# jaak-s/libfastsparse

Measured on AMD Instinct MI355X. Metric: fp64 CSR SpMV effective GB/s (% HBM3E peak), higher is better.
Workload: dtype f64

## Files before the change

libfastsparse_amd/csrc/fs_kernels_twopass.hip:

```cpp
#include <stdlib.h>

#include "fs_kernel_util.h"

namespace fs {


template <int U, bool NTLD, bool NTST, int BC>
__device__ __forceinline__ void expand_share(double *__restrict__ xband, int ncol, int B, const unsigned *__restrict__ band_ptr,
                                             const uint16_t *__restrict__ lcol, const unsigned *__restrict__ gdst,
                                             const double *__restrict__ x, int xs, double *__restrict__ prod, unsigned g0,
                                             unsigned g1)
{
  const int t = threadIdx.x;
  if (g0 >= g1) return;
  int b;
  {
    int lo = 0, hi = B - 1;
    while (lo < hi) {
      const int mid = lo + ((hi - lo + 1) >> 1);
      if (band_ptr[mid] <= g0) lo = mid; else hi = mid - 1;
    }
    b = lo;
  }
  for (unsigned g = g0; g < g1; ++b) {
    const unsigned gb = band_ptr[b + 1] < g1 ? band_ptr[b + 1] : g1;
    if (gb <= g) continue;
    const int c0 = b * BC;
    const int w = (ncol - c0 < BC) ? ncol - c0 : BC;
    __syncthreads();
    {
      double r[BC / kBinBlock];
#pragma unroll
      for (int j = 0; j < BC / kBinBlock; ++j) {
        const int i = j * kBinBlock + t;
        r[j] = __builtin_nontemporal_load(x + (int64_t)(c0 + (i < w ? i : w - 1)) * xs);
      }
#pragma unroll
      for (int j = 0; j < BC / kBinBlock; ++j) {
        const int i = j * kBinBlock + t;
        xband[i] = (i < w) ? r[j] : 0.0;
      }
      if (t < 8) xband[BC + t] = 0.0;
    }
    __syncthreads();
    const int64_t e0 = (int64_t)g * kBinGroup, e1 = (int64_t)gb * kBinGroup;
    constexpr int64_t kRound = 2 * U * kBinBlock;
    int64_t o = e0 + 2 * t;
    for (; o - 2 * t + kRound <= e1; o += kRound) {
      unsigned a[U], d[U];
#pragma unroll
      for (int k = 0; k < U; ++k) {
        const int64_t e = o + (int64_t)k * 2 * kBinBlock;
        a[k] = stream_load<NTLD>((const unsigned *)(lcol + e));
        d[k] = stream_load<NTLD>(gdst + (e >> kBinGroupLog));
      }
      __builtin_amdgcn_sched_barrier(0);
#pragma unroll
      for (int k = 0; k < U; ++k) {
        const int64_t e = o + (int64_t)k * 2 * kBinBlock;
        const v2d p = {xband[a[k] & 0xffffu], xband[a[k] >> 16]};
        stream_store<NTST>(p, (v2d *)(prod + (int64_t)d[k] * kBinGroup + (e & (kBinGroup - 1))));
      }
    }
    for (; o < e1; o += 2 * kBinBlock) {
      const unsigned a = stream_load<NTLD>((const unsigned *)(lcol + o));
      const unsigned d = stream_load<NTLD>(gdst + (o >> kBinGroupLog));
      const v2d p = {xband[a & 0xffffu], xband[a >> 16]};
      stream_store<NTST>(p, (v2d *)(prod + (int64_t)d * kBinGroup + (o & (kBinGroup - 1))));
    }
    g = gb;
  }
}

template <int U, bool NTLD, bool NTST, int BC = kBinCols>
__global__ __launch_bounds__(kBinBlock) void spmv_expand_kernel(
    int ncol, int B, const unsigned *__restrict__ band_ptr, const uint16_t *__restrict__ lcol,
    const unsigned *__restrict__ gdst, const double *__restrict__ x, int xs, double *__restrict__ prod, unsigned gbeg,
    unsigned gend)
{
  __shared__ double xband[BC + 8];
  const uint64_t groups = gend - gbeg;
  const unsigned g0 = gbeg + (unsigned)(groups * blockIdx.x / gridDim.x), g1 = gbeg + (unsigned)(groups * (blockIdx.x + 1) / gridDim.x);
  expand_share<U, NTLD, NTST, BC>(xband, ncol, B, band_ptr, lcol, gdst, x, xs, prod, g0, g1);
}

static_assert(kBinGroupLog == 4, "the one-byte row ids (row_ids, line_ids, rows8_decode_kernel) decode groups of 16 entries: two lanes of 8, eight lanes of 2, four words of 4");
template <bool NTLD, bool L8>
__device__ __forceinline__ v4u row_ids_load(const uint16_t *__restrict__ lrow, const uint8_t *__restrict__ lrow8,
                                            const uint16_t *__restrict__ gbase, int64_t e)
{
  if (!L8) return stream_load<NTLD>((const v4u *)(lrow + e));
  typedef unsigned v2u __attribute__((ext_vector_type(2)));
  const v2u d = stream_load<NTLD>((const v2u *)(lrow8 + e));
  return v4u{d.x, d.y, (unsigned)gbase[e >> kBinGroupLog], (unsigned)(e >> 3) & 1u};
}

template <bool L8>
__device__ __forceinline__ v4u row_ids(v4u raw)
{
  if (!L8) return raw;
  const unsigned dx = raw.x, dy = raw.y;
  const unsigned s0 = dx & 0xffu, s1 = s0 + ((dx >> 8) & 0xffu), s2 = s1 + ((dx >> 16) & 0xffu), s3 = s2 + (dx >> 24);
  const unsigned s4 = s3 + (dy & 0xffu), s5 = s4 + ((dy >> 8) & 0xffu), s6 = s5 + ((dy >> 16) & 0xffu), s7 = s6 + (dy >> 24);
  const unsigned below = (unsigned)__builtin_amdgcn_update_dpp(0, (int)s7, 0x111 , 0xf, 0xf, false);
  const unsigned off = raw.z + (raw.w ? below : 0u);
  return v4u{(off + s0) | ((off + s1) << 16), (off + s2) | ((off + s3) << 16), (off + s4) | ((off + s5) << 16), (off + s6) | ((off + s7) << 16)};
}

template <bool L8>
__device__ __forceinline__ unsigned line_ids_load(const uint16_t *__restrict__ lrow, const uint8_t *__restrict__ lrow8,
                                                  const uint16_t *__restrict__ gbase, int64_t e)
{
  if (!L8) return *(const unsigned *)(lrow + e);
  return (unsigned)*(const uint16_t *)(lrow8 + e) | ((unsigned)gbase[e >> kBinGroupLog] << 16);
}

template <bool L8>
__device__ __forceinline__ unsigned line_ids(unsigned raw)
{
  if (!L8) return raw;
  const unsigned d0 = raw & 0xffu, own = d0 + ((raw >> 8) & 0xffu), l = threadIdx.x & 7u;
  unsigned s = own, u;
  u = (unsigned)__builtin_amdgcn_update_dpp(0, (int)s, 0x111 , 0xf, 0xf, false); s += l >= 1 ? u : 0u;
  u = (unsigned)__builtin_amdgcn_update_dpp(0, (int)s, 0x112 , 0xf, 0xf, false); s += l >= 2 ? u : 0u;
  u = (unsigned)__builtin_amdgcn_update_dpp(0, (int)s, 0x114 , 0xf, 0xf, false); s += l >= 4 ? u : 0u;
  const unsigned off = (raw >> 16) + s - own;
  return (off + d0) | ((off + own) << 16);
}

template <bool VALUED, bool NTLD, bool L8 = false>
__device__ __forceinline__ void reduce_panel(double *__restrict__ ytile, int panel, const unsigned *__restrict__ bin_ptr,
                                             const int *__restrict__ panel_row, const uint16_t *__restrict__ lrow,
                                             const double *__restrict__ vals, const double *__restrict__ prod, double *__restrict__ y,
                                             int ys, const uint8_t *__restrict__ lrow8 = nullptr,
                                             const uint16_t *__restrict__ gbase = nullptr)
{
  const int t = threadIdx.x;
  const int r0 = panel_row[panel], nr = panel_row[panel + 1] - r0;
  for (int i = t; i < nr; i += kBinBlock) ytile[i] = 0.0;
  __syncthreads();
  const int64_t e0 = (int64_t)bin_ptr[panel] * kBinGroup, e1 = (int64_t)bin_ptr[panel + 1] * kBinGroup;
#define FS_ADD(idx, val) __hip_atomic_fetch_add(&ytile[idx], val, __ATOMIC_RELAXED, __HIP_MEMORY_SCOPE_WORKGROUP)
#define FS_ADD2(A, P) FS_ADD((A) & 0xffffu, (P).x); FS_ADD((A) >> 16, (P).y);
  constexpr int64_t kStep = 8 * kBinBlock, kRound = 2 * kStep;
  const int wave0 = (t >> 6) * 512, lane0 = wave0 + 2 * (t & 63);
  int64_t eb = e0;
  for (; eb + kRound <= e1; eb += kRound) {
    const int64_t e = eb + lane0;
    unsigned a[2][4];
    v2d p[2][4], v[2][4];
#pragma unroll
    for (int k = 0; k < 2; ++k)
#pragma unroll
      for (int j = 0; j < 4; ++j) {
        const int64_t ek = e + k * kStep + 128 * j;
        a[k][j] = line_ids_load<L8>(lrow, lrow8, gbase, ek);
        p[k][j] = stream_load<NTLD>((const v2d *)(prod + ek));
        if (VALUED) v[k][j] = stream_load<NTLD>((const v2d *)(vals + ek));
      }
    __builtin_amdgcn_sched_barrier(0);
#pragma unroll
    for (int k = 0; k < 2; ++k)
#pragma unroll
      for (int j = 0; j < 4; ++j) {
        const unsigned r = line_ids<L8>(a[k][j]);
        if (VALUED) { p[k][j].x *= v[k][j].x; p[k][j].y *= v[k][j].y; }
        FS_ADD2(r, p[k][j])
      }
  }
  for (; eb + wave0 < e1; eb += kStep) {
    const int64_t e = eb + lane0;
    unsigned a[4];
    v2d p[4], v[4];
#pragma unroll
    for (int j = 0; j < 4; ++j) {
      const int64_t ej = e + 128 * j, ec = ej < e1 ? ej : e1 - 2;
      a[j] = line_ids_load<L8>(lrow, lrow8, gbase, ec);
      p[j] = stream_load<NTLD>((const v2d *)(prod + ec));
      if (VALUED) v[j] = stream_load<NTLD>((const v2d *)(vals + ec));
    }
#pragma unroll
    for (int j = 0; j < 4; ++j) {
      const unsigned r = line_ids<L8>(a[j]);
      if (VALUED) { p[j].x *= v[j].x; p[j].y *= v[j].y; }
      if (e + 128 * j < e1) { FS_ADD2(r, p[j]) }
    }
  }
#undef FS_ADD2
#undef FS_ADD
  __syncthreads();
  for (int i = t; i < nr; i += kBinBlock) y[(int64_t)(r0 + i) * ys] = ytile[i];
}

template <bool VALUED, bool NTLD, int RM = kBinRowsMax, bool L8 = false>
__global__ __launch_bounds__(kBinBlock) void spmv_reduce_kernel(
    const unsigned *__restrict__ bin_ptr, const int *__restrict__ panel_row, const uint16_t *__restrict__ lrow,
    const double *__restrict__ vals, const double *__restrict__ prod, double *__restrict__ y, int ys, int pbase,
    const uint8_t *__restrict__ lrow8 = nullptr, const uint16_t *__restrict__ gbase = nullptr)
{
  __shared__ double ytile[RM];
  reduce_panel<VALUED, NTLD, L8>(ytile, pbase + blockIdx.x, bin_ptr, panel_row, lrow, vals, prod, y, ys, lrow8, gbase);
}

#ifndef FS_ORDERED_DEPTH
#define FS_ORDERED_DEPTH 16
#endif
#ifndef FS_ORDERED_DEPTH_VALUED
#define FS_ORDERED_DEPTH_VALUED 10
#endif
template <bool VALUED, bool NTLD, int RM, int DEPTH, bool L8 = false>
__global__ __launch_bounds__(64) void spmv_reduce_ordered_kernel(
    const unsigned *__restrict__ bin_ptr, const int *__restrict__ panel_row, const uint16_t *__restrict__ lrow,
    const double *__restrict__ vals, const double *__restrict__ prod, double *__restrict__ y, int ys, int pbase,
    const uint8_t *__restrict__ lrow8 = nullptr, const uint16_t *__restrict__ gbase = nullptr)
{
  __shared__ __attribute__((aligned(16))) double ytile[RM];
  const int t = threadIdx.x;
  const int panel = pbase + blockIdx.x;
  const int r0 = panel_row[panel], nr = panel_row[panel + 1] - r0;
  for (int i = 2 * t; i < nr; i += 128) *reinterpret_cast<v2d *>(&ytile[i]) = v2d{0.0, 0.0};
  const int64_t e0 = (int64_t)bin_ptr[panel] * kBinGroup, e1 = (int64_t)bin_ptr[panel + 1] * kBinGroup;
#define FS_ADD(idx, val) __hip_atomic_fetch_add(&ytile[idx], val, __ATOMIC_RELAXED, __HIP_MEMORY_SCOPE_WORKGROUP)
#define FS_ADD8(A, P)                                                  \
  FS_ADD(A.x & 0xffffu, P[0].x); FS_ADD(A.x >> 16, P[0].y);            \
  FS_ADD(A.y & 0xffffu, P[1].x); FS_ADD(A.y >> 16, P[1].y);            \
  FS_ADD(A.z & 0xffffu, P[2].x); FS_ADD(A.z >> 16, P[2].y);            \
  FS_ADD(A.w & 0xffffu, P[3].x); FS_ADD(A.w >> 16, P[3].y);
  constexpr int64_t kStep = 8 * 64;
  v4u a[DEPTH];
  v2d p[DEPTH][4], v[VALUED ? DEPTH : 1][4];
  auto fetch = [&](int k, int64_t e) {
    const int64_t ec = (e + 8 <= e1) ? e : (e1 - e0 >= 8 ? e1 - 8 : e0);
    a[k] = row_ids_load<NTLD, L8>(lrow, lrow8, gbase, ec);
#pragma unroll
    for (int j = 0; j < 4; ++j) {
      p[k][j] = stream_load<NTLD>((const v2d *)(prod + ec + 2 * j));
      if (VALUED) v[k][j] = stream_load<NTLD>((const v2d *)(vals + ec + 2 * j));
    }
  };
  if (e1 > e0) {
    int64_t e = e0 + 8 * t;
#pragma unroll
    for (int k = 0; k < DEPTH; ++k) fetch(k, e + (int64_t)k * kStep);
    for (; e - 8 * t < e1; e += (int64_t)DEPTH * kStep) {
#pragma unroll
      for (int k = 0; k < DEPTH; ++k) {
        const int64_t ek = e + (int64_t)k * kStep;
        const v4u ak = row_ids<L8>(a[k]);
        v2d pk[4] = {p[k][0], p[k][1], p[k][2], p[k][3]};
        if (VALUED) {
#pragma unroll
          for (int j = 0; j < 4; ++j) { pk[j].x *= v[k][j].x; pk[j].y *= v[k][j].y; }
        }
        fetch(k, ek + (int64_t)DEPTH * kStep);
        if (ek + 8 <= e1) { FS_ADD8(ak, pk) }
      }
    }
  }
#undef FS_ADD8
#undef FS_ADD
  __syncthreads();
  for (int i = t; i < nr; i += 64) y[(int64_t)(r0 + i) * ys] = ytile[i];
}

template <bool VALUED, int BC, int NACC, bool ORDERED>
__global__ __launch_bounds__(kBinBlock) void spmv_longrows_kernel(
    int ncol, int B, int nlong, const int64_t *__restrict__ band_ptr, const unsigned *__restrict__ seg_ptr,
    const uint16_t *__restrict__ lcol, const uint16_t *__restrict__ lrow, const double *__restrict__ vals,
    const double *__restrict__ x, int xs, double *__restrict__ ylong, double *__restrict__ ypart)
{
  __shared__ double xband[BC + 8];
  __shared__ double acc[NACC];
  const int t = threadIdx.x, lane = t & 63, wave = t >> 6;
  for (int i = t; i < nlong; i += kBinBlock) acc[i] = 0.0;
  const int64_t pairs = band_ptr[B] >> 1;
  const int64_t e_beg = 2 * (pairs * blockIdx.x / gridDim.x), e_end = 2 * (pairs * (blockIdx.x + 1) / gridDim.x);
  if (e_beg < e_end) {
    int b;
    {
      int lo = 0, hi = B - 1;
      while (lo < hi) {
        const int mid = lo + ((hi - lo + 1) >> 1);
        if (band_ptr[mid] <= e_beg) lo = mid; else hi = mid - 1;
      }
      b = lo;
    }
    double rn[BC / kBinBlock];
    int have = -1;
    auto request = [&](int bb) {
      const int cb = bb * BC;
      const int wb = (ncol - cb < BC) ? ncol - cb : BC;
#pragma unroll
      for (int j = 0; j < BC / kBinBlock; ++j) {
        const int i = j * kBinBlock + t;
        rn[j] = __builtin_nontemporal_load(x + (int64_t)(cb + (i < wb ? i : wb - 1)) * xs);
      }
      have = bb;
    };
    auto wave_step = [&](int64_t o, bool live, int64_t oc) {
      const unsigned a = *reinterpret_cast<const unsigned *>(lcol + oc);
      const unsigned rr = *reinterpret_cast<const unsigned *>(lrow + oc);
      v2d p = {xband[a & 0xffffu], xband[a >> 16]};
      if (VALUED) { const v2d v = *reinterpret_cast<const v2d *>(vals + oc); p.x *= v.x; p.y *= v.y; }
      unsigned key = 0xffffffffu;
      double sum = 0.0;
      if (live) {
        const unsigned r0 = rr & 0xffffu, r1 = rr >> 16;
        if (r0 == r1) { key = r0; sum = p.x + p.y; }
        else { __hip_atomic_fetch_add(&acc[r0], p.x, __ATOMIC_RELAXED, __HIP_MEMORY_SCOPE_WORKGROUP); key = r1; sum = p.y; }
      }
#pragma unroll
      for (int d = 1; d < 64; d <<= 1) {
        const unsigned ku = __shfl_up(key, d);
        const double su = __shfl_up(sum, d);
        if (lane >= d && ku == key) sum += su;
      }
      const unsigned kn = __shfl_down(key, 1);
      if (live && (lane == 63 || kn != key))
        __hip_atomic_fetch_add(&acc[key], sum, __ATOMIC_RELAXED, __HIP_MEMORY_SCOPE_WORKGROUP);
      (void)o;
    };
    for (int64_t e = e_beg; e < e_end; ++b) {
      const int64_t eb = band_ptr[b + 1] < e_end ? band_ptr[b + 1] : e_end;
      if (eb <= e) continue;
      const int c0 = b * BC;
      const int w = (ncol - c0 < BC) ? ncol - c0 : BC;
      if (have != b) request(b);
      __syncthreads();
#pragma unroll
      for (int j = 0; j < BC / kBinBlock; ++j) {
        const int i = j * kBinBlock + t;
        xband[i] = (i < w) ? rn[j] : 0.0;
      }
      if (t < 8) xband[BC + t] = 0.0;
      __syncthreads();
      if (b + 1 < B && eb < e_end) request(b + 1);
      if (ORDERED) {
        const int64_t s0 = band_ptr[b] + seg_ptr[b * (kLongOwners + 1) + wave], s1 = band_ptr[b] + seg_ptr[b * (kLongOwners + 1) + wave + 1];
        const int64_t lo = s0 > e ? s0 : e, hi = s1 < eb ? s1 : eb;
        for (int64_t o0 = lo; o0 < hi; o0 += 128) {
          const int64_t o = o0 + 2 * lane;
          const bool live = o < hi;
          wave_step(o, live, live ? o : lo);
        }
      } else {
        for (int64_t o0 = e; o0 < eb; o0 += 2 * kBinBlock) {
          const int64_t o = o0 + 2 * t;
          const bool live = o < eb;
          wave_step(o, live, live ? o : e);
        }
      }
      e = eb;
    }
  }
  __syncthreads();
  if (ORDERED) {
    double *__restrict__ mine = ypart + (int64_t)blockIdx.x * nlong;
    for (int i = t; i < nlong; i += kBinBlock) mine[i] = acc[i];
  } else {
    for (int i = t; i < nlong; i += kBinBlock) {
      const double v = acc[i];
      if (v != 0.0) unsafeAtomicAdd(ylong + i, v);
    }
  }
}

__global__ __launch_bounds__(kBlock) void longrows_combine_kernel(int nlong, int nwg, const double *__restrict__ ypart, double *__restrict__ ylong)
{
  const int i = blockIdx.x * kBlock + threadIdx.x;
  if (i >= nlong) return;
  double acc = 0.0;
  for (int w = 0; w < nwg; ++w) acc += ypart[(int64_t)w * nlong + i];
  ylong[i] = acc;
}

__global__ __launch_bounds__(kBlock) void longrows_scatter_kernel(int nlong, const int *__restrict__ row, const double *__restrict__ ylong,
                                                                 double *__restrict__ y, int ys, int row0, int row1)
{
  const int i = blockIdx.x * kBlock + threadIdx.x;
  if (i >= nlong) return;
  const int r = row[i];
  if (r >= row0 && r < row1) y[(int64_t)r * ys] = 0.0 + ylong[i];
}

static int launch_longrows(const DeviceCsr &A, const LongRows &L, const double *x, int xs, hipStream_t s)
{
  const bool ordered = reproducible_now();
  if (!ordered || L.n == 0 || L.nwg == 0)
    if (int rc = launch_zero(L.ylong, sizeof(double) * (size_t)L.nlong, s)) return rc;
  if (L.n == 0 || L.nwg == 0) return FS_OK;
#define FS_LONG(V, BC, NA, ORD)                                                                                              \
  hipLaunchKernelGGL((spmv_longrows_kernel<V, BC, NA, ORD>), dim3(L.nwg), dim3(kBinBlock), 0, s, A.ncol, L.B, L.nlong, L.band_ptr, \
                     L.seg_ptr, L.lcol, L.lrow, L.vals, x, xs, L.ylong, L.ypart)
#define FS_LONG2(V, BC, NA) do { if (ordered) FS_LONG(V, BC, NA, true); else FS_LONG(V, BC, NA, false); } while (0)
  if (L.bcols == kLongBandB) { if (A.has_vals()) FS_LONG2(true, kLongBandB, kLongRowsB); else FS_LONG2(false, kLongBandB, kLongRowsB); }
  else                       { if (A.has_vals()) FS_LONG2(true, kLongBandA, kLongRowsA); else FS_LONG2(false, kLongBandA, kLongRowsA); }
#undef FS_LONG2
#undef FS_LONG
  FS_HIP(hipGetLastError());
  if (ordered) {
    hipLaunchKernelGGL(longrows_combine_kernel, dim3((unsigned)((L.nlong + kBlock - 1) / kBlock)), dim3(kBlock), 0, s, L.nlong, L.nwg, L.ypart,
                       L.ylong);
    FS_HIP(hipGetLastError());
  }
  return FS_OK;
}


template <int K, int U>
__global__ __launch_bounds__(kBinBlock) void spmm_expand_kernel(
    int ncol, int B, const unsigned *__restrict__ band_ptr, const uint16_t *__restrict__ lcol,
    const unsigned *__restrict__ gdst, const double *__restrict__ X, int xs, double *__restrict__ prod)
{
  constexpr int BC = kBinCols / K;
  constexpr int GE = kBinGroup / K;
  constexpr int LP = K / 2;
  constexpr int EPS = kBinBlock / LP;
  __shared__ __attribute__((aligned(16))) double xband[kBinCols + 8];
  const int t = threadIdx.x;
  const int le = t / LP, h = t % LP;
  const uint64_t groups = band_ptr[B];
  const unsigned g0 = (unsigned)(groups * blockIdx.x / gridDim.x), g1 = (unsigned)(groups * (blockIdx.x + 1) / gridDim.x);
  if (g0 >= g1) return;
  int b;
  {
    int lo = 0, hi = B - 1;
    while (lo < hi) {
      const int mid = lo + ((hi - lo + 1) >> 1);
      if (band_ptr[mid] <= g0) lo = mid; else hi = mid - 1;
    }
    b = lo;
  }
  for (unsigned g = g0; g < g1; ++b) {
    const unsigned gb = band_ptr[b + 1] < g1 ? band_ptr[b + 1] : g1;
    if (gb <= g) continue;
    const int c0 = b * BC;
    const int w = (ncol - c0 < BC) ? ncol - c0 : BC;
    __syncthreads();
    {
      double r[kBinCols / kBinBlock];
#pragma unroll
      for (int j = 0; j < kBinCols / kBinBlock; ++j) {
        const int f = j * kBinBlock + t, i = f / K, q = f % K;
        r[j] = __builtin_nontemporal_load(X + (int64_t)(c0 + (i < w ? i : w - 1)) * xs + q);
      }
#pragma unroll
      for (int j = 0; j < kBinCols / kBinBlock; ++j) {
        const int f = j * kBinBlock + t;
        xband[f] = (f / K < w) ? r[j] : 0.0;
      }
      if (t < 8) xband[kBinCols + t] = 0.0;
    }
    __syncthreads();
    const int64_t e0 = (int64_t)g * GE, e1 = (int64_t)gb * GE;
    constexpr int64_t kRound = (int64_t)U * EPS;
    int64_t o = e0 + le;
    for (; o - le + kRound <= e1; o += kRound) {
      unsigned a[U], d[U];
#pragma unroll
      for (int k = 0; k < U; ++k) {
        const int64_t e = o + (int64_t)k * EPS;
        a[k] = lcol[e];
        d[k] = gdst[e / GE];
      }
      __builtin_amdgcn_sched_barrier(0);
#pragma unroll
      for (int k = 0; k < U; ++k) {
        const int64_t e = o + (int64_t)k * EPS;
        const v2d p = *reinterpret_cast<const v2d *>(&xband[a[k] * K + 2 * h]);
        __builtin_nontemporal_store(p, (v2d *)(prod + ((int64_t)d[k] * GE + (e % GE)) * K + 2 * h));
      }
    }
    for (; o < e1; o += EPS) {
      const unsigned a = lcol[o];
      const unsigned d = gdst[o / GE];
      const v2d p = *reinterpret_cast<const v2d *>(&xband[a * K + 2 * h]);
      __builtin_nontemporal_store(p, (v2d *)(prod + ((int64_t)d * GE + (o % GE)) * K + 2 * h));
    }
    g = gb;
  }
}

template <bool VALUED, int K>
__global__ __launch_bounds__(kBinBlock) void spmm_reduce_kernel(
    const unsigned *__restrict__ bin_ptr_all, const int *__restrict__ panel_row_all, const uint16_t *__restrict__ lrow,
    const double *__restrict__ vals, const double *__restrict__ prod, double *__restrict__ Y, int ys, int pbase)
{
  const unsigned *__restrict__ bin_ptr = bin_ptr_all + pbase;
  const int *__restrict__ panel_row = panel_row_all + pbase;
  constexpr int GE = kBinGroup / K;
  constexpr int EPL = 8 / K;
  __shared__ double ytile[kBinRowsMax];
  const int t = threadIdx.x;
  const int r0 = panel_row[blockIdx.x], nr = panel_row[blockIdx.x + 1] - r0;
  for (int i = t; i < nr * K; i += kBinBlock) ytile[i] = 0.0;
  __syncthreads();
  const int64_t e0 = (int64_t)bin_ptr[blockIdx.x] * GE, e1 = (int64_t)bin_ptr[blockIdx.x + 1] * GE;
  typedef uint16_t rows_t __attribute__((ext_vector_type(EPL)));
  typedef double vals_t __attribute__((ext_vector_type(EPL)));
#define FS_ADD(idx, val) __hip_atomic_fetch_add(&ytile[idx], val, __ATOMIC_RELAXED, __HIP_MEMORY_SCOPE_WORKGROUP)
  auto add8 = [&](const rows_t a, const v2d (&p)[4], const vals_t v) {
#pragma unroll
    for (int q = 0; q < EPL; ++q) {
      const int base = (int)a[q] * K;
#pragma unroll
      for (int j = 0; j < K; j += 2) {
        v2d t2 = p[(q * K + j) / 2];
        if (VALUED) { t2.x *= v[q]; t2.y *= v[q]; }
        FS_ADD(base + j, t2.x);
        FS_ADD(base + j + 1, t2.y);
      }
    }
  };
  constexpr int64_t kStep = (int64_t)EPL * kBinBlock;
  constexpr int64_t kRound = 2 * kStep;
  int64_t e = e0 + (int64_t)EPL * t;
  for (; e - EPL * t + kRound <= e1; e += kRound) {
    rows_t a[2];
    v2d p[2][4];
    vals_t v[2] = {};
#pragma unroll
    for (int k = 0; k < 2; ++k) {
      const int64_t ek = e + k * kStep;
      a[k] = *reinterpret_cast<const rows_t *>(lrow + ek);
      if (VALUED) v[k] = *reinterpret_cast<const vals_t *>(vals + ek);
#pragma unroll
      for (int j = 0; j < 4; ++j) p[k][j] = *reinterpret_cast<const v2d *>(prod + ek * K + 2 * j);
    }
    __builtin_amdgcn_sched_barrier(0);
    add8(a[0], p[0], v[0]);
    add8(a[1], p[1], v[1]);
  }
  for (; e < e1; e += kStep) {
    const rows_t a = *reinterpret_cast<const rows_t *>(lrow + e);
    vals_t v = {};
    if (VALUED) v = *reinterpret_cast<const vals_t *>(vals + e);
    v2d p[4];
#pragma unroll
    for (int j = 0; j < 4; ++j) p[j] = *reinterpret_cast<const v2d *>(prod + e * K + 2 * j);
    add8(a, p, v);
  }
#undef FS_ADD
  __syncthreads();
  for (int i = t; i < nr * K; i += kBinBlock) Y[(int64_t)(r0 + i / K) * ys + (i % K)] = ytile[i];
}

template <bool VALUED, int K, int DEPTH>
__global__ __launch_bounds__(64) void spmm_reduce_ordered_kernel(
    const unsigned *__restrict__ bin_ptr_all, const int *__restrict__ panel_row_all, const uint16_t *__restrict__ lrow,
    const double *__restrict__ vals, const double *__restrict__ prod, double *__restrict__ Y, int ys, int pbase)
{
  const unsigned *__restrict__ bin_ptr = bin_ptr_all + pbase;
  const int *__restrict__ panel_row = panel_row_all + pbase;
  constexpr int GE = kBinGroup / K;
  constexpr int EPL = 8 / K;
  __shared__ double ytile[kBinRowsMax];
  const int t = threadIdx.x;
  const int r0 = panel_row[blockIdx.x], nr = panel_row[blockIdx.x + 1] - r0;
  for (int i = t; i < nr * K; i += 64) ytile[i] = 0.0;
  const int64_t e0 = (int64_t)bin_ptr[blockIdx.x] * GE, e1 = (int64_t)bin_ptr[blockIdx.x + 1] * GE;
  typedef uint16_t rows_t __attribute__((ext_vector_type(EPL)));
  typedef double vals_t __attribute__((ext_vector_type(EPL)));
#define FS_ADD(idx, val) __hip_atomic_fetch_add(&ytile[idx], val, __ATOMIC_RELAXED, __HIP_MEMORY_SCOPE_WORKGROUP)
  auto add8 = [&](const rows_t a, const v2d (&p)[4], const vals_t v) {
#pragma unroll
    for (int q = 0; q < EPL; ++q) {
      const int base = (int)a[q] * K;
#pragma unroll
      for (int j = 0; j < K; j += 2) {
        v2d t2 = p[(q * K + j) / 2];
        if (VALUED) { t2.x *= v[q]; t2.y *= v[q]; }
        FS_ADD(base + j, t2.x);
        FS_ADD(base + j + 1, t2.y);
      }
    }
  };
  constexpr int64_t kStep = (int64_t)EPL * 64;
  rows_t a[DEPTH];
  v2d p[DEPTH][4];
  vals_t v[VALUED ? DEPTH : 1] = {};
  auto fetch = [&](int k, int64_t e) {
    const int64_t ec = (e + EPL <= e1) ? e : (e1 - e0 >= EPL ? e1 - EPL : e0);
    a[k] = *reinterpret_cast<const rows_t *>(lrow + ec);
    if (VALUED) v[k] = *reinterpret_cast<const vals_t *>(vals + ec);
#pragma unroll
    for (int j = 0; j < 4; ++j) p[k][j] = *reinterpret_cast<const v2d *>(prod + ec * K + 2 * j);
  };
  if (e1 > e0) {
    int64_t e = e0 + (int64_t)EPL * t;
#pragma unroll
    for (int k = 0; k < DEPTH; ++k) fetch(k, e + (int64_t)k * kStep);
    for (; e - EPL * t < e1; e += (int64_t)DEPTH * kStep) {
#pragma unroll
      for (int k = 0; k < DEPTH; ++k) {
        const int64_t ek = e + (int64_t)k * kStep;
        const rows_t ak = a[k];
        const v2d pk[4] = {p[k][0], p[k][1], p[k][2], p[k][3]};
        const vals_t vk = v[VALUED ? k : 0];
        fetch(k, ek + (int64_t)DEPTH * kStep);
        if (ek + EPL <= e1) add8(ak, pk, vk);
      }
    }
  }
#undef FS_ADD
  __syncthreads();
  for (int i = t; i < nr * K; i += 64) Y[(int64_t)(r0 + i / K) * ys + (i % K)] = ytile[i];
}

template <int K>
__global__ __launch_bounds__(kBlock) void tiled_combine_k_kernel(int nrow, const int *__restrict__ vfirst,
                                                                const double *__restrict__ yv, double *__restrict__ Y, int ys,
                                                                int row0 = 0)
{
  const int64_t i = (int64_t)row0 * K + (int64_t)blockIdx.x * kBlock + threadIdx.x;
  const int64_t r = i / K;
  const int j = (int)(i % K);
  if (r >= nrow) return;
  const int a = vfirst[r], b = vfirst[r + 1];
  double acc = yv[(int64_t)a * K + j];
  for (int v = a + 1; v < b; ++v) acc += yv[(int64_t)v * K + j];
  Y[r * ys + j] = acc;
}

__global__ void rows8_decode_kernel(int64_t groups, const uint8_t *__restrict__ lrow8, const uint16_t *__restrict__ gbase,
                                    uint16_t *__restrict__ lrow)
{
  const int64_t g = (int64_t)blockIdx.x * blockDim.x + threadIdx.x;
  if (g >= groups) return;
  const v4u d = *(const v4u *)(lrow8 + g * kBinGroup);
  unsigned r = gbase[g];
  unsigned out[kBinGroup / 2];
#pragma unroll
  for (int j = 0; j < kBinGroup; j += 2) {
    const unsigned w = j < 4 ? d.x : j < 8 ? d.y : j < 12 ? d.z : d.w;
    const unsigned a = r + ((w >> (8 * (j & 3))) & 0xffu), b = a + ((w >> (8 * ((j + 1) & 3))) & 0xffu);
    out[j / 2] = a | (b << 16);
    r = b;
  }
#pragma unroll
  for (int j = 0; j < kBinGroup / 8; ++j)
    *(v4u *)(lrow + g * kBinGroup + 8 * j) = v4u{out[4 * j], out[4 * j + 1], out[4 * j + 2], out[4 * j + 3]};
}

static void ensure_two_byte_ids(BinnedCsr &N, hipStream_t s)
{
  if (N.lrow || !N.lrow8 || N.lrow_tried) return;
  hipStreamCaptureStatus cap = hipStreamCaptureStatusNone;
  if (hipStreamIsCapturing(s, &cap) != hipSuccess) { (void)hipGetLastError(); return; }
  if (cap != hipStreamCaptureStatusNone) return;
  N.lrow_tried = true;
  uint16_t *p = nullptr;
  if (hipMalloc(&p, sizeof(uint16_t) * (size_t)N.n) != hipSuccess) { (void)hipGetLastError(); return; }
  const int64_t groups = N.n >> kBinGroupLog;
  if (groups > 0) hipLaunchKernelGGL(rows8_decode_kernel, dim3((unsigned)((groups + 255) / 256)), dim3(256), 0, s, groups, N.lrow8, N.gbase, p);
  if (hipGetLastError() != hipSuccess || hipStreamSynchronize(s) != hipSuccess) { (void)hipGetLastError(); (void)hipFree(p); return; }
  N.lrow = p;
}

static void launch_reduce(const BinnedCsr &N, double *out, int os, int p0, int p1, int flags, hipStream_t s)
{
#define FS_REDUCE(V, NT, RM, L8)                                                                                                \
  hipLaunchKernelGGL((spmv_reduce_kernel<V, NT, RM, L8>), dim3(p1 - p0), dim3(kBinBlock), 0, s, N.bin_ptr, N.panel_row, N.lrow, \
                     N.vals, N.prod, out, os, p0, N.lrow8, N.gbase)
#define FS_REDUCE2(RM, L8)                                                                       \
  do {                                                                                           \
    if (N.vals) { if (flags & 256) FS_REDUCE(true, false, RM, L8); else FS_REDUCE(true, true, RM, L8); }   \
    else        { if (flags & 256) FS_REDUCE(false, false, RM, L8); else FS_REDUCE(false, true, RM, L8); } \
  } while (0)
  if (N.bcols == kBinColsBig) FS_REDUCE2(kBinRowsBig, false);
  else if (N.lrow8)           FS_REDUCE2(kBinRowsMax, true);
  else                        FS_REDUCE2(kBinRowsMax, false);
#undef FS_REDUCE2
#undef FS_REDUCE
}

int launch_spmv_binned(const DeviceCsr &A, double *y, const double *x, hipStream_t s, int xs, int ys, int p0, int p1, int row0,
                       int row1)
{
  const BinnedCsr &N = *A.binned;
  double *out = N.split ? N.yv : y;
  const int os = N.split ? 1 : ys;
  const bool part = p1 >= 0;
  if (!part) { p0 = 0; p1 = N.P; row0 = 0; row1 = A.nrow; }
  const int nwg1 = (options().bin_wgs > 0 && options().bin_wgs < N.nwg1) ? options().bin_wgs : N.nwg1;
  if (nwg1 > 0 && p0 == 0) {
    const int flags = options().bin_flags;
#define FS_EXPAND4(U)                                                                                       \
  do {                                                                                                      \
    if (flags & 16) { if (flags & 8) FS_EXPAND(U, true, false);  else FS_EXPAND(U, true, true); }           \
    else            { if (flags & 8) FS_EXPAND(U, false, false); else FS_EXPAND(U, false, true); }          \
  } while (0)
#define FS_EXPAND(U, NL, NS)                                                                                      \
  hipLaunchKernelGGL((spmv_expand_kernel<U, NL, NS>), dim3(nwg1), dim3(kBinBlock), 0, s, A.ncol, N.B, N.band_ptr, \
                     N.lcol, N.gdst, x, xs, N.prod, 0u, (unsigned)(N.n >> kBinGroupLog))
    if (N.bcols == kBinColsBig)
      hipLaunchKernelGGL((spmv_expand_kernel<4, false, true, kBinColsBig>), dim3(nwg1), dim3(kBinBlock), 0, s, A.ncol, N.B,
                         N.band_ptr, N.lcol, N.gdst, x, xs, N.prod, 0u, (unsigned)(N.n >> kBinGroupLog));
    else if ((flags & 3) == 1) FS_EXPAND4(8);
    else if ((flags & 3) == 2) FS_EXPAND4(2);
    else                       FS_EXPAND4(4);
#undef FS_EXPAND4
#undef FS_EXPAND
    FS_HIP(hipGetLastError());
  }
  if (N.lr && p0 == 0)
    if (int rc = launch_longrows(A, *N.lr, x, xs, s)) return rc;
  if (p1 > p0) {
    const bool ordered = reproducible_now() || (options().bin_flags & 32);
    if (ordered && N.lrow8 && !N.lrow) ensure_two_byte_ids(*A.binned, s);
#define FS_ORDERED(RM, L8)                                                                                                     \
  do {                                                                                                                         \
    if (N.vals)                                                                                                                \
      hipLaunchKernelGGL((spmv_reduce_ordered_kernel<true, false, RM, FS_ORDERED_DEPTH_VALUED, L8>), dim3(p1 - p0), dim3(64), 0, s, \
                         N.bin_ptr, N.panel_row, N.lrow, N.vals, N.prod, out, os, p0, N.lrow8, N.gbase);                       \
    else                                                                                                                       \
      hipLaunchKernelGGL((spmv_reduce_ordered_kernel<false, false, RM, FS_ORDERED_DEPTH, L8>), dim3(p1 - p0), dim3(64), 0, s,  \
                         N.bin_ptr, N.panel_row, N.lrow, N.vals, N.prod, out, os, p0, N.lrow8, N.gbase);                       \
  } while (0)
    if (N.bcols == kBinColsBig && ordered)  FS_ORDERED(kBinRowsBig, false);
    else if (ordered && N.lrow8 && !N.lrow) FS_ORDERED(kBinRowsMax, true);
    else if (ordered)                       FS_ORDERED(kBinRowsMax, false);
    else
      launch_reduce(N, out, os, p0, p1, options().bin_flags, s);
#undef FS_ORDERED
    FS_HIP(hipGetLastError());
  }
  if (N.split && row1 > row0) {
    if (int rc = launch_tiled_combine(row1, N.vfirst, N.yv, y, ys, row0, s)) return rc;
  }
  if (N.lr && row1 > row0) {
    hipLaunchKernelGGL(longrows_scatter_kernel, dim3((unsigned)((N.lr->nlong + kBlock - 1) / kBlock)), dim3(kBlock), 0, s, N.lr->nlong,
                       N.lr->row, N.lr->ylong, y, ys, row0, row1);
    FS_HIP(hipGetLastError());
  }
  return FS_OK;
}

int launch_expand_groups(const DeviceCsr &A, const double *x, unsigned g0, unsigned g1, int wgs, hipStream_t s)
{
  const BinnedCsr &N = *A.binned;
  if (g1 <= g0 || wgs <= 0) return FS_OK;
#define FS_XH(BC)                                                                                                         \
  hipLaunchKernelGGL((spmv_expand_kernel<4, false, true, BC>), dim3(wgs), dim3(kBinBlock), 0, s, A.ncol, N.B, N.band_ptr, \
                     N.lcol, N.gdst, x, 1, N.prod, g0, g1)
  if (N.bcols == kBinColsBig) FS_XH(kBinColsBig);
  else                        FS_XH(kBinCols);
#undef FS_XH
  FS_HIP(hipGetLastError());
  return FS_OK;
}

int launch_reduce_panels(const DeviceCsr &A, double *y, int p0, int p1, hipStream_t s)
{
  const BinnedCsr &N = *A.binned;
  if (p1 <= p0) return FS_OK;
  launch_reduce(N, y, 1, p0, p1, 0, s);
  FS_HIP(hipGetLastError());
  return FS_OK;
}

int launch_spmm_binned(const DeviceCsr &A, const BinnedCsr &N, double *Y, const double *X, hipStream_t s, int xs, int ys, int p0,
                       int p1, int row0, int row1)
{
  const int K = N.kw;
  double *out = N.split ? N.yv : Y;
  const int os = N.split ? K : ys;
  if (p1 < 0) { p0 = 0; p1 = N.P; row0 = 0; row1 = A.nrow; }
  const int nwg1 = (p0 != 0) ? 0 : ((options().bin_wgs > 0 && options().bin_wgs < N.nwg1) ? options().bin_wgs : N.nwg1);
#define FS_XP(KK)                                                                                                  \
  hipLaunchKernelGGL((spmm_expand_kernel<KK, 4>), dim3(nwg1), dim3(kBinBlock), 0, s, A.ncol, N.B, N.band_ptr, N.lcol, \
                     N.gdst, X, xs, N.prod)
  if (nwg1 > 0) {
    if (K == 2) FS_XP(2); else FS_XP(4);
    FS_HIP(hipGetLastError());
  }
#undef FS_XP
  if (p1 > p0) {
    const bool ordered = reproducible_now() || (options().bin_flags & 32);
#define FS_RP(V, KK)                                                                                                            \
  do {                                                                                                                          \
    if (ordered)                                                                                                                \
      hipLaunchKernelGGL((spmm_reduce_ordered_kernel<V, KK, (V && KK == 2) ? 12 : FS_ORDERED_DEPTH>), dim3(p1 - p0), dim3(64), 0, s, N.bin_ptr, \
                         N.panel_row, N.lrow, N.vals, N.prod, out, os, p0);                                                     \
    else                                                                                                                        \
      hipLaunchKernelGGL((spmm_reduce_kernel<V, KK>), dim3(p1 - p0), dim3(kBinBlock), 0, s, N.bin_ptr, N.panel_row, N.lrow,     \
                         N.vals, N.prod, out, os, p0);                                                                          \
  } while (0)
    if (K == 2) { if (N.vals) FS_RP(true, 2); else FS_RP(false, 2); }
    else        { if (N.vals) FS_RP(true, 4); else FS_RP(false, 4); }
#undef FS_RP
    FS_HIP(hipGetLastError());
  }
  if (N.split && row1 > row0) {
    const unsigned grid = (unsigned)(((int64_t)(row1 - row0) * K + kBlock - 1) / kBlock);
    if (K == 2)
      hipLaunchKernelGGL(tiled_combine_k_kernel<2>, dim3(grid), dim3(kBlock), 0, s, row1, N.vfirst, N.yv, Y, ys, row0);
    else
      hipLaunchKernelGGL(tiled_combine_k_kernel<4>, dim3(grid), dim3(kBlock), 0, s, row1, N.vfirst, N.yv, Y, ys, row0);
    FS_HIP(hipGetLastError());
  }
  return FS_OK;
}

}
```

Before: 2676.

## Add producer-consumer feeder waves for ordered SpMV reduce via LDS ring

Adds a reduce kernel for the ordered (reproducible) path in which extra feeder waves stream product and value arrays, multiply them, and write into a double-buffered shared-memory ring. A single adder wave consumes the ring and does the LDS atomic adds in a fixed order. The aim is to split memory streaming from the serialized accumulation so that HBM loads overlap the ordered adds. It adds block-wide barriers per ring half and only runs when ordered mode is active and values are present, or when a flag enables it.

Result: slower. 2644 (-1.2%).

```diff
diff --git a/libfastsparse_amd/csrc/fs_kernels_twopass.hip b/libfastsparse_amd/csrc/fs_kernels_twopass.hip
--- a/libfastsparse_amd/csrc/fs_kernels_twopass.hip
+++ b/libfastsparse_amd/csrc/fs_kernels_twopass.hip
@@ -261,6 +261,125 @@
 #undef FS_ADD
   __syncthreads();
   for (int i = t; i < nr; i += 64) y[(int64_t)(r0 + i) * ys] = ytile[i];
+}
+
+constexpr int kRingSteps = 8, kRingPart = 4;
+#ifndef FS_ORDERED_FEEDERS
+#define FS_ORDERED_FEEDERS 2
+#endif
+#ifndef FS_ORDERED_FEEDER_STEPS
+#define FS_ORDERED_FEEDER_STEPS 8
+#endif
+#ifndef FS_ORDERED_ADDER_PARTS
+#define FS_ORDERED_ADDER_PARTS (FS_ORDERED_DEPTH / kRingPart)
+#endif
+template <bool VALUED, int W, int PF, int PA, bool L8 = false>
+__global__ __launch_bounds__(64 * (1 + W)) void spmv_reduce_ordered_feeders_kernel(
+    const unsigned *__restrict__ bin_ptr, const int *__restrict__ panel_row, const uint16_t *__restrict__ lrow,
+    const double *__restrict__ vals, const double *__restrict__ prod, double *__restrict__ y, int ys, int pbase,
+    const uint8_t *__restrict__ lrow8 = nullptr, const uint16_t *__restrict__ gbase = nullptr)
+{
+  static_assert(kRingSteps == 2 * kRingPart && kRingPart % W == 0, "two ring parts, each a whole number of steps per feeder");
+  static_assert(PF >= 1 && PF * kRingPart == FS_ORDERED_FEEDER_STEPS * W, "a feeder's steps in flight are whole ring parts");
+  constexpr int S = kRingPart, SW = S / W;
+  constexpr int64_t kStep = 8 * 64;
+  __shared__ __attribute__((aligned(16))) double ytile[kBinRowsMax];
+  __shared__ v2d ring[kRingSteps * 256];
+  const int t = threadIdx.x, lane = t & 63;
+  const int wave = __builtin_amdgcn_readfirstlane(t >> 6);
+  const int panel = pbase + blockIdx.x;
+  const int r0 = panel_row[panel], nr = panel_row[panel + 1] - r0;
+  for (int i = 2 * t; i < nr; i += 128 * (1 + W)) *reinterpret_cast<v2d *>(&ytile[i]) = v2d{0.0, 0.0};
+  const int64_t e0 = (int64_t)bin_ptr[panel] * kBinGroup, e1 = (int64_t)bin_ptr[panel + 1] * kBinGroup;
+  constexpr int R = PA > PF ? PA : PF;
+  static_assert(R % PA == 0 && R % PF == 0, "a round is whole turns of both prefetch rings");
+  const int parts = (int)((e1 - e0 + R * S * kStep - 1) / (R * S * kStep)) * R;
+  if (wave == 0) {
+#define FS_ADD(idx, val) __hip_atomic_fetch_add(&ytile[idx], val, __ATOMIC_RELAXED, __HIP_MEMORY_SCOPE_WORKGROUP)
+#define FS_ADD8(A, P)                                                  \
+  FS_ADD(A.x & 0xffffu, P[0].x); FS_ADD(A.x >> 16, P[0].y);            \
+  FS_ADD(A.y & 0xffffu, P[1].x); FS_ADD(A.y >> 16, P[1].y);            \
+  FS_ADD(A.z & 0xffffu, P[2].x); FS_ADD(A.z >> 16, P[2].y);            \
+  FS_ADD(A.w & 0xffffu, P[3].x); FS_ADD(A.w >> 16, P[3].y);
+    v4u a[PA * S];
+    const int64_t elane = e0 + 8 * lane;
+    auto fetch = [&](int k, int g) {
+      const int64_t e = elane + g * kStep;
+      a[k] = row_ids_load<false, L8>(lrow, lrow8, gbase, (e + 8 <= e1) ? e : e1 - 8);
+    };
+    if (parts > 0) {
+#pragma unroll
+      for (int k = 0; k < PA * S; ++k) fetch(k, k);
+    }
+    for (int q0 = 0; q0 < parts; q0 += PA) {
+#pragma unroll
+      for (int i = 0; i < PA; ++i) {
+        const int q = q0 + i;
+        {
+          __syncthreads();
+          const v2d *half = ring + (q & 1) * (S * 256);
+          v2d pk[S][4];
+#pragma unroll
+          for (int u = 0; u < S; ++u)
+#pragma unroll
+            for (int jj = 0; jj < 4; ++jj) pk[u][jj] = half[u * 256 + jj * 64 + (lane ^ (2 * jj))];
+#pragma unroll
+          for (int u = 0; u < S; ++u) {
+            const int g = q * S + u;
+            const v4u ak = row_ids<L8>(a[i * S + u]);
+            fetch(i * S + u, g + PA * S);
+            if (elane + g * kStep + 8 <= e1) { FS_ADD8(ak, pk[u]) }
+          }
+        }
+      }
+    }
+#undef FS_ADD8
+#undef FS_ADD
+  } else {
+    const int f = wave - 1;
+    v2d p[PF * SW][4], v[VALUED ? PF * SW : 1][4];
+    const int64_t elane = e0 + 2 * lane;
+    auto fetch = [&](int k, int g) {
+#pragma unroll
+      for (int j = 0; j < 4; ++j) {
+        const int64_t e = elane + g * kStep + 128 * j, ec = e < e1 ? e : e1 - 2;
+        p[k][j] = stream_load<true>((const v2d *)(prod + ec));
+        if (VALUED) v[k][j] = stream_load<true>((const v2d *)(vals + ec));
+      }
+    };
+    const int cell = (lane & 3) * 64 + ((lane >> 2) ^ (2 * (lane & 3)));
+    if (parts > 0) {
+#pragma unroll
+      for (int i = 0; i < PF; ++i)
+#pragma unroll
+        for (int u = 0; u < SW; ++u) fetch(i * SW + u, i * S + u * W + f);
+    }
+    for (int q0 = 0; q0 < parts; q0 += PF) {
+#pragma unroll
+      for (int i = 0; i < PF; ++i) {
+        const int q = q0 + i;
+        {
+          v2d *half = ring + (q & 1) * (S * 256) + cell;
+#pragma unroll
+          for (int u = 0; u < SW; ++u) {
+            const int k = i * SW + u, s = u * W + f;
+            __builtin_amdgcn_sched_barrier(0);
+            v2d pk[4] = {p[k][0], p[k][1], p[k][2], p[k][3]};
+            if (VALUED) {
+#pragma unroll
+              for (int j = 0; j < 4; ++j) { pk[j].x *= v[k][j].x; pk[j].y *= v[k][j].y; }
+            }
+            fetch(k, (q + PF) * S + s);
+#pragma unroll
+            for (int j = 0; j < 4; ++j) half[s * 256 + 16 * j] = pk[j];
+          }
+          __syncthreads();
+        }
+      }
+    }
+  }
+  __syncthreads();
+  for (int i = t; i < nr; i += 64 * (1 + W)) y[(int64_t)(r0 + i) * ys] = ytile[i];
 }
 
 template <bool VALUED, int BC, int NACC, bool ORDERED>
@@ -717,7 +836,21 @@
       hipLaunchKernelGGL((spmv_reduce_ordered_kernel<false, false, RM, FS_ORDERED_DEPTH, L8>), dim3(p1 - p0), dim3(64), 0, s,  \
                          N.bin_ptr, N.panel_row, N.lrow, N.vals, N.prod, out, os, p0, N.lrow8, N.gbase);                       \
   } while (0)
-    if (N.bcols == kBinColsBig && ordered)  FS_ORDERED(kBinRowsBig, false);
+#define FS_FEEDERS(V, WW, L8)                                                                                                  \
+  hipLaunchKernelGGL((spmv_reduce_ordered_feeders_kernel<V, (WW), FS_ORDERED_FEEDER_STEPS * (WW) / kRingPart, FS_ORDERED_ADDER_PARTS, L8>), \
+                     dim3(p1 - p0), dim3(64 * (1 + (WW))), 0, s, N.bin_ptr, N.panel_row, N.lrow, N.vals, N.prod, out, os, p0,    \
+                     N.lrow8, N.gbase)
+#define FS_FEEDERS2(L8)                                                                                                        \
+  do {                                                                                                                         \
+    const bool other = (fflags & 1024) != 0;                                                                                   \
+    if (N.vals) { if (other) FS_FEEDERS(true, 3 - FS_ORDERED_FEEDERS, L8); else FS_FEEDERS(true, FS_ORDERED_FEEDERS, L8); }    \
+    else        { if (other) FS_FEEDERS(false, 3 - FS_ORDERED_FEEDERS, L8); else FS_FEEDERS(false, FS_ORDERED_FEEDERS, L8); }  \
+  } while (0)
+    const int fflags = options().bin_flags;
+    const bool feeders = ordered && N.bcols != kBinColsBig && !(fflags & 512) && (N.vals || (fflags & 2048));
+    if (feeders && N.lrow8 && !N.lrow)      FS_FEEDERS2(true);
+    else if (feeders)                       FS_FEEDERS2(false);
+    else if (N.bcols == kBinColsBig && ordered)  FS_ORDERED(kBinRowsBig, false);
     else if (ordered && N.lrow8 && !N.lrow) FS_ORDERED(kBinRowsMax, true);
     else if (ordered)                       FS_ORDERED(kBinRowsMax, false);
     else
```
